# HelixDB/helix-db

Hardware: AMD Instinct MI355X
Metric: QPS @ recall@10>=0.95, 1Mx768 fp32; achieved HBM GB/s vs roofline (higher is better)
Workload: dtype f32; 1 GPU; configs[1]: 1000000x768 f32 per GPU, HNSW M=16/M0=32 ef_search=128 k=10, batch=1024 queries, squared-L2, strict-exhaustive beam (bit-exact vs reference CPU path), steps issued round-robin on 4 execution lanes; dataset=embedding, rows_per_gpu=1000000, rows_total=1000000, dim=768, batch=1024, k=10, ef_search=128, lanes=4, distinct_query_batches=25, exchange=single GPU, parallelism=1 GPU

## Files before the change

### helix-db_amd/csrc/hvx_api.hip

```cpp
#include <hip/hip_runtime.h>

#include <algorithm>
#include <atomic>
#include <cmath>
#include <cstdarg>
#include <cstdio>
#include <cstdlib>
#include <cstring>
#include <mutex>
#include <string>
#include <thread>
#include <vector>

#include "hvx_host.h"
#include "hvx_flat_mfma.h"
#include "hvx_hnsw_plan.h"

using namespace hvx;

namespace {
thread_local std::string g_err;
}

namespace hvx {
// ... 691 lines not shown
        return HVX_OK;
    }
    HIP_TRY(launch_validate_queries(ix->dev, d_queries, b, ix->limit, ix->d_qstatus, ix->d_qhdr, ix->stream));
    HnswArgs a;
    a.ix = ix->dev;
    a.queries = d_queries;
    a.qstatus = ix->d_qstatus;
    a.qhdr = ix->d_qhdr;
    a.bitmap = ix->d_bitmap;
    a.bitmap2 = (ad && ad->count_reads) ? ix->d_bitmap2 : nullptr;
    a.words_per_query = ix->words_per_query;
    a.k = k;
    a.ef = ef;
    a.out_ids = d_ids;
    a.out_scores = d_scores;
    a.out_counts = d_counts;
    a.out_status = d_status;
    a.qstats = d_qstats ? d_qstats : ix->d_qstats;
    a.tie_flags = ix->d_tie;
    a.rerun_list = ix->d_tie + ix->max_batch;
    a.rerun_ctl = ix->d_tie + 2 * (size_t)ix->max_batch;
    a.prof = nullptr;
    a.wave_clock = nullptr;
    a.adaptive = ad ? 1u : 0u;
    a.ad = ad ? *ad : AdaptArgs{};
    a.build_nodes = nullptr;
    a.build_ef_upper = 0;
    a.only_flagged = 0;
    a.occupancy = ix->occupancy;
    a.pair = ix->opt[HVX_OPT_HNSW_PAIR] >= 2u || (ix->opt[HVX_OPT_HNSW_PAIR] == 0u && ix->occupancy != 2u) ? 1u : 0u;
    a.pair_gatherers = ix->opt[HVX_OPT_HNSW_PAIR] == 3u ? 1u : 0u;
    a.log2cap = ix->opt[HVX_OPT_WAVE_LOG2CAP];
    a.shadow = nullptr;
    a.shadow_err = nullptr;
    if (ad) {
        if (!hnsw_wave_adaptive_supported(a))
            return fail(HVX_ERR_UNSUPPORTED, "the non-strict search arms serve f32 rows of any dimension / metric (bf16 rows: dim in "
                        "{128,256,384,512,768,1024,1536}, cosine / Euclidean), neighbour rows <= 64 ids, ef <= 800");
        if (ix->bitmap_dirty) {
            HIP_TRY(hipMemsetAsync(ix->d_bitmap, 0, (size_t)ix->max_batch * ix->words_per_query * 4, ix->stream));
            ix->bitmap_dirty = false;
        }
        const bool ad_prof = tuning_env("HVX_WAVE_PROF") != nullptr && hnsw_wave_supported(a) && ix->occupancy != 2u;
        if (ad_prof) {
            if (!ix->d_prof && ix->dalloc((void **)&ix->d_prof, (size_t)ix->max_batch * 80)) return HVX_ERR_DEVICE;
            a.prof = ix->d_prof;
        }
        hipEvent_t e0 = nullptr, e1 = nullptr;
        pick_events(ix, timed, &e0, &e1, &a.wave_clock);
        if (e0) HIP_TRY(hipEventRecord(e0, ix->stream));
        HIP_TRY(launch_hnsw_wave(a, b, ix->stream));
        if (e1) HIP_TRY(hipEventRecord(e1, ix->stream));
        if (ad_prof) {
            std::vector<unsigned long long> h((size_t)b * 10);
            HIP_TRY(hipMemcpyAsync(h.data(), ix->d_prof, h.size() * 8, hipMemcpyDeviceToHost, ix->stream));
            HIP_TRY(hipStreamSynchronize(ix->stream));
            double acc[10] = {0, 0, 0, 0, 0, 0, 0, 0, 0, 0};
            for (uint32_t i = 0; i < b; ++i)
                for (int j = 0; j < 10; ++j) acc[j] += (double)h[(size_t)i * 10 + j];
            fprintf(stderr, "[hvx prof, non-strict] per query: row-wait %.0f  visited-claim %.0f  decide+select %.0f  gather+fma %.0f  predict %.0f  admit %.0f  (layer-0 loop %.0f) cycles\n",
                    acc[0] / b, acc[1] / b, acc[6] / b, acc[2] / b, acc[3] / b, acc[4] / b, acc[7] / b);
        }
        return HVX_OK;
    }
    const bool prof = tuning_env("HVX_WAVE_PROF") != nullptr;
    if (prof) {
        if (!ix->d_prof && ix->dalloc((void **)&ix->d_prof, (size_t)ix->max_batch * 80)) return HVX_ERR_DEVICE;
        a.prof = ix->d_prof;
    }
    const bool force_general = ix->opt[HVX_OPT_HNSW_GENERAL_KERNEL] != 0;
    const bool wave = !(force_general && ix->dev.dtype == HVX_F32) && hnsw_wave_supported(a);
    if (!wave && ix->dev.dtype != HVX_F32)
        return fail(HVX_ERR_UNSUPPORTED, ix->dev.dtype == HVX_FP8_E4M3 ? "fp8 rows serve the exact scan only (HNSW over fp8 rows is not built)"
                    : "bf16 rows are served by the one-wavefront-per-query kernel only (dim in {128,256,384,512,768,1024,1536}, rows <= 64 ids, ef <= 800)");
    if (ix->bitmap_dirty) {
        HIP_TRY(hipMemsetAsync(ix->d_bitmap, 0, (size_t)ix->max_batch * ix->words_per_query * 4, ix->stream));
        ix->bitmap_dirty = false;
    }
    if (wave && (ix->occupancy == 2 || prof) && ix->dev.dtype == HVX_F32 && ix->dev.metric == kL2 && !ix->opt[HVX_OPT_HNSW_SHADOW_PRUNE]) {
        uint16_t *sh = nullptr;
        float *se = nullptr;
        int rc = shadow_catch_up(ix, &sh, &se);
        if (rc) return rc;
        a.shadow = sh;
        a.shadow_err = se;
    }
    hipEvent_t e0 = nullptr, e1 = nullptr;
    pick_events(ix, timed, &e0, &e1, &a.wave_clock);
    if (e0) HIP_TRY(hipEventRecord(e0, ix->stream));
    if (wave) {
        HIP_TRY(launch_hnsw_wave(a, b, ix->stream));
        if (prof) {
            std::vector<unsigned long long> h((size_t)b * 10);
            HIP_TRY(hipMemcpyAsync(h.data(), ix->d_prof, h.size() * 8, hipMemcpyDeviceToHost, ix->stream));
            HIP_TRY(hipStreamSynchronize(ix->stream));
            double acc[10] = {0, 0, 0, 0, 0, 0, 0, 0, 0, 0};
            for (uint32_t i = 0; i < b; ++i)
                for (int j = 0; j < 10; ++j) acc[j] += (double)h[(size_t)i * 10 + j];
            fprintf(stderr, "[hvx prof] per query: row-wait %.0f  visited+shadow %.0f  gather+fma %.0f  predict %.0f  admit %.0f  (layer-0 loop %.0f) cycles;"
                            " fresh-candidate predictions %.1f  row-prefetch hits %.1f;  full-beam rows: shadow-pruned %.1f  scored in f32 %.1f"
                            " (pruned share %.4f)\n",
                    acc[0] / b, acc[1] / b, acc[2] / b, acc[3] / b, acc[4] / b, acc[7] / b, acc[5] / b, acc[6] / b, acc[8] / b, acc[9] / b,
                    acc[8] + acc[9] > 0 ? acc[8] / (acc[8] + acc[9]) : 0.0);
        }
    } else {
        HIP_TRY(launch_hnsw_search(a, b, ix->stream));
        ix->bitmap_dirty = true;
    }
    if (e1) HIP_TRY(hipEventRecord(e1, ix->stream));
    return HVX_OK;
}

extern "C" int hvx_index_timing_begin(hvx_index *ix, uint32_t capacity) {
    if (!ix) return fail(HVX_ERR_INVARIANT, "null index");
    std::lock_guard<std::mutex> lock(ix->mu);
    HIP_TRY(hipSetDevice(ix->device));
    while (ix->ring.size() < (size_t)capacity * 2) {
        hipEvent_t e;
// ... 334 lines not shown
```

### helix-db_amd/csrc/hvx_flat_mfma.hip

```cpp
#include <hip/hip_runtime.h>

#include <algorithm>
#include <vector>

#include "hvx_hnsw_wave.h"
#include "hvx_host.h"
#include "hvx_flat_mfma.h"

using namespace hvx;

#define HIP_TRY(expr)                                                                              \
    do {                                                                                           \
        hipError_t _e = (expr);                                                                    \
        if (_e != hipSuccess) return fail(HVX_ERR_DEVICE, "%s: %s", #expr, hipGetErrorString(_e)); \
    } while (0)

namespace hvx {

constexpr int HVX_MFMA_FALLBACK = -1;

typedef __attribute__((ext_vector_type(8))) __bf16 bf16x8;
typedef __attribute__((ext_vector_type(16))) float f32x16;

__global__ __launch_bounds__(64) void bf16_row_norm2_kernel(const uint16_t *rows, uint32_t n, uint32_t dim, float *out) {
    const uint32_t r = blockIdx.x;
    if (r >= n) return;
    const uint16_t *p = rows + (size_t)r * dim;
    double acc = 0.0;
    for (uint32_t i = threadIdx.x; i < dim; i += 64) {
        const double v = (double)bf16_to_f32(p[i]);
        acc += v * v;
    }
    for (int s = 32; s > 0; s >>= 1) acc += __shfl_xor(acc, s, 64);
    if (threadIdx.x == 0) out[r] = (float)acc;
}

__global__ __launch_bounds__(64) void fp8_code_norm_kernel(const uint8_t *codes, uint32_t n, uint32_t dim, float *out) {
    const uint32_t r = blockIdx.x;
    if (r >= n) return;
    const uint8_t *p = codes + (size_t)r * dim;
    double acc = 0.0;
    for (uint32_t i = threadIdx.x; i < dim; i += 64) {
        const double v = (double)fp8_e4m3_decode(p[i]);
        acc += v * v;
    }
    for (int s = 32; s > 0; s >>= 1) acc += __shfl_xor(acc, s, 64);
    if (threadIdx.x == 0) out[r] = (float)sqrt(acc);
}

__global__ __launch_bounds__(256) void bf16_shadow_kernel(const float *rows, uint32_t ld, uint32_t dim, size_t cnt, uint16_t *out, float *err) {
    const uint32_t lane = threadIdx.x & 63u;
    for (size_t r = (size_t)blockIdx.x * 4 + (threadIdx.x >> 6); r < cnt; r += (size_t)gridDim.x * 4) {
        const float *x = rows + r * ld;
        uint16_t *o = out + r * dim;
        double acc = 0.0;
        if ((dim & 3u) == 0u) {
            for (uint32_t i = lane; i < dim / 4u; i += 64u) {
                const float4 v = reinterpret_cast<const float4 *>(x)[i];
                const uint32_t a = f32_to_bf16_rne(v.x), b = f32_to_bf16_rne(v.y), c = f32_to_bf16_rne(v.z), d = f32_to_bf16_rne(v.w);
                reinterpret_cast<uint2 *>(o)[i] = make_uint2(a | (b << 16), c | (d << 16));
                const double ea = (double)v.x - (double)bf16_to_f32((uint16_t)a), eb = (double)v.y - (double)bf16_to_f32((uint16_t)b);
                const double ec = (double)v.z - (double)bf16_to_f32((uint16_t)c), ed = (double)v.w - (double)bf16_to_f32((uint16_t)d);
                acc += ea * ea + eb * eb + ec * ec + ed * ed;
            }
        } else {
            for (uint32_t i = lane; i < dim; i += 64u) {
                const uint16_t h = f32_to_bf16_rne(x[i]);
                o[i] = h;
                const double ei = (double)x[i] - (double)bf16_to_f32(h);
                acc += ei * ei;
            }
        }
        for (int s = 32; s > 0; s >>= 1) acc += __shfl_xor(acc, s, 64);
        if (lane == 0u) {
            const double e = sqrt(acc) * (1.0 + 0x1p-30);
            float f = (float)e;
            if ((double)f < e) f = __uint_as_float(__float_as_uint(f) + 1u);
            err[r] = f;
        }
    }
}

__global__ __launch_bounds__(64) void split_queries_kernel(const float *q, uint32_t b, uint32_t bpad, uint32_t dim,
                                                           uint16_t *qhi, uint16_t *qlo, float *qn2, uint32_t fp8_layout,
                                                           uint16_t *qhi_tile8, uint32_t cosine) {
    const uint32_t r = blockIdx.x;
    if (r >= bpad) return;
    int qe = 0;
    if (cosine && r < b) {
        float mx = 0.f;
        for (uint32_t i = threadIdx.x; i < dim; i += 64) {
            const float v = q[(size_t)r * dim + i];
            if (f32_is_finite(v)) mx = fmaxf(mx, fabsf(v));
        }
        for (int s = 32; s > 0; s >>= 1) mx = fmaxf(mx, __shfl_xor(mx, s, 64));
        qe = cosine_query_exponent(mx);
    }
    double acc = 0.0;
    for (uint32_t i = threadIdx.x; i < dim; i += 64) {
        float v = r < b ? q[(size_t)r * dim + i] : 0.f;
        if (!f32_is_finite(v)) v = 0.f;
        if (qe) v = ldexpf(v, -qe);
        const uint16_t h = f32_to_bf16_rne(v);
        const float res = v - bf16_to_f32(h);
        const uint32_t s = fp8_layout == 2u ? i : (fp8_layout ? fp8_slot_of(i) : bf16_slot_of(i));
        qhi[(size_t)r * dim + s] = h;
        qlo[(size_t)r * dim + s] = f32_to_bf16_rne(res);
        if (qhi_tile8) qhi_tile8[(size_t)r * dim + tile_slot_fp8(s)] = h;
        acc += (double)v * (double)v;
    }
    for (int s = 32; s > 0; s >>= 1) acc += __shfl_xor(acc, s, 64);
    if (threadIdx.x == 0 && r < b) qn2[r] = (float)acc;
// ... 510 lines not shown
            const float t = t_thr;
            const float e = METRIC == kL2 ? a.erel * 0.5f * (a.qn2[q] + a.xmax2) : a.erel;
            const float kth = outn ? ss[outn - 1] : inf;
            ok = (outn == a.k && kth < t - e) ? 1u : 0u;
        }
        a.cert[q] = ok;
    }
}

template <uint32_t METRIC>
static hipError_t launch_rerank(const RerankArgs &a, uint32_t b, hipStream_t s) {
    const size_t lds = (size_t)a.ix.dim * 4 + 8192 + (a.sl_sc ? (size_t)a.sl_n * 4 : 0);
    switch (a.ix.dim >> 5) {
#define HVX_RR(N)                                                                                                   \
    case N:                                                                                                         \
        if (a.ix.dtype == HVX_FP8_E4M3) hipLaunchKernelGGL((rerank_bf16_kernel<METRIC, N, 1>), dim3(b), dim3(256), lds, s, a); \
        else if (a.ix.dtype == HVX_F32) hipLaunchKernelGGL((rerank_bf16_kernel<METRIC, N, 2>), dim3(b), dim3(256), lds, s, a);  \
        else hipLaunchKernelGGL((rerank_bf16_kernel<METRIC, N, 0>), dim3(b), dim3(256), lds, s, a);                  \
        break;
        HVX_RR(4) HVX_RR(8) HVX_RR(16) HVX_RR(24) HVX_RR(32) HVX_RR(48)
#undef HVX_RR
    default: return hipErrorInvalidValue;
    }
    return hipGetLastError();
}

}

extern "C" float hvxi_scan_error_bound(uint32_t kind, uint32_t l2, uint32_t dim) { return hvx::scan_error_bound(kind, l2 != 0u, dim); }
extern "C" int hvxi_cosine_query_exponent(float mx) { return hvx::cosine_query_exponent(mx); }
extern "C" uint32_t hvxi_cosine_term_trusted(float term) { return hvx::cosine_term_trusted(term) ? 1u : 0u; }

namespace hvx {

hipError_t launch_fp8_code_norm(const uint8_t *codes, uint32_t n, uint32_t dim, float *out, hipStream_t s) {
    if (n == 0) return hipSuccess;
    hipLaunchKernelGGL(fp8_code_norm_kernel, dim3(n), dim3(64), 0, s, codes, n, dim, out);
    return hipGetLastError();
}

hipError_t launch_bf16_row_norm2(const uint16_t *rows, uint32_t n, uint32_t dim, float *out, hipStream_t s) {
    if (n == 0) return hipSuccess;
    hipLaunchKernelGGL(bf16_row_norm2_kernel, dim3(n), dim3(64), 0, s, rows, n, dim, out);
    return hipGetLastError();
}

static int flat_mfma_impl(hvx_index *ix, const float *d_queries, uint32_t b, uint32_t k, const uint32_t *d_subset, uint32_t n_rows,
                          uint64_t *d_ids, float *d_scores, uint32_t *d_counts, uint32_t *d_status, bool timed, bool allow_filter,
                          bool force_tail = false);

int flat_mfma_device(hvx_index *ix, const float *d_queries, uint32_t b, uint32_t k, const uint32_t *d_subset, uint32_t n_rows,
                     uint64_t *d_ids, float *d_scores, uint32_t *d_counts, uint32_t *d_status, bool timed) {
    return flat_mfma_impl(ix, d_queries, b, k, d_subset, n_rows, d_ids, d_scores, d_counts, d_status, timed, true);
}

int shadow_catch_up(hvx_index *ix, uint16_t **shadow, float **err) {
    const DevIndex &d = ix->dev;
    hvx_image_shared &sh = *ix->shared;
    std::lock_guard<std::mutex> lock(sh.mu);
    *shadow = nullptr;
    *err = nullptr;
    if (sh.shadow_failed) return HVX_OK;
    if (!sh.shadow) {
        void *p = nullptr;
        const size_t rows_cap = std::max<uint64_t>(ix->cap_rows, d.n);
        const size_t sbytes = (rows_cap * d.dim * 2 + 15) / 16 * 16;
        if (hipMalloc(&p, std::max<size_t>(sbytes + rows_cap * 4, 16)) != hipSuccess) {
            (void)hipGetLastError();
            sh.shadow_failed = true;
            return HVX_OK;
        }
        sh.device = ix->device;
        sh.shadow = reinterpret_cast<uint16_t *>(p);
        sh.shadow_err = reinterpret_cast<float *>(reinterpret_cast<char *>(p) + sbytes);
        sh.shadow_rows = 0;
    }
    if (sh.shadow_rows < d.n) {
        const size_t r0 = sh.shadow_rows, cnt = d.n - r0;
        const uint32_t blocks = (uint32_t)std::min<size_t>((cnt + 3) / 4, 4096);
        hipLaunchKernelGGL(bf16_shadow_kernel, dim3(blocks), dim3(256), 0, ix->stream, d.vec + r0 * d.ld, d.ld, d.dim, cnt, sh.shadow + r0 * d.dim,
                           sh.shadow_err + r0);
        if (hipGetLastError() != hipSuccess || hipStreamSynchronize(ix->stream) != hipSuccess) return fail(HVX_ERR_DEVICE, "bf16 shadow conversion failed");
        sh.shadow_rows = d.n;
    }
    *shadow = sh.shadow;
    *err = sh.shadow_err;
    return HVX_OK;
}
static int ensure_shadow(hvx_index *ix) {
    uint16_t *s = nullptr;
    float *e = nullptr;
    const int rc = shadow_catch_up(ix, &s, &e);
    ix->m_shadow = s;
    return rc;
}

static int flat_mfma_impl(hvx_index *ix, const float *d_queries, uint32_t b, uint32_t k, const uint32_t *d_subset, uint32_t n_rows,
                          uint64_t *d_ids, float *d_scores, uint32_t *d_counts, uint32_t *d_status, bool timed, bool allow_filter,
                          bool force_tail) {
    const DevIndex &d = ix->dev;
    const uint32_t n = n_rows;
    if (k == 0) return fail(HVX_ERR_K_RANGE, "result count must be non-zero");
    if (k > 511) return fail(HVX_ERR_UNSUPPORTED, "bf16 exact scan supports k <= 511");
    const uint32_t nk = d.dim >> 5;
    if (nk != 4 && nk != 8 && nk != 16 && nk != 24 && nk != 32 && nk != 48)
        return fail(HVX_ERR_UNSUPPORTED, "bf16 / fp8 exact scan serves dim in {128,256,512,768,1024,1536}");
    HIP_TRY(launch_validate_queries(d, d_queries, b, ix->limit, ix->d_qstatus, ix->d_qhdr, ix->stream));
    if (n == 0) {
        if (timed) {
            HIP_TRY(hipEventRecord(ix->ev0, ix->stream));
            HIP_TRY(hipEventRecord(ix->ev1, ix->stream));
        }
        HIP_TRY(hipMemsetAsync(d_counts, 0, (size_t)b * 4, ix->stream));
        if (d_status) HIP_TRY(hipMemcpyAsync(d_status, ix->d_qstatus, (size_t)b * 4, hipMemcpyDeviceToDevice, ix->stream));
        return HVX_OK;
    }
    const uint32_t bpad = (b + 255u) / 256u * 256u;
    int rc;
    const bool fp8 = d.dtype == HVX_FP8_E4M3, f32 = d.dtype == HVX_F32;
    if ((size_t)bpad * d.dim > ix->cap_qsplit) {
        if ((rc = ix->regrow((void **)&ix->m_qhi, (size_t)bpad * d.dim * 2))) return rc;
        if ((rc = ix->regrow((void **)&ix->m_qlo, (size_t)bpad * d.dim * 2))) return rc;
        if (fp8 && (rc = ix->regrow((void **)&ix->m_qhi8, (size_t)bpad * d.dim * 2))) return rc;
        if ((rc = ix->regrow((void **)&ix->m_qn2, (size_t)bpad * 4))) return rc;
// ... 246 lines not shown
```

### helix-db_amd/csrc/hvx_hnsw_wave.h

```cpp
#pragma once
#include <type_traits>

#include "hvx_beam.h"
#include "hvx_device.h"
#include "hvx_hnsw_plan.h"
#include "hvx_kernels.h"
#include "hvx_shadow_bound.h"

namespace hvx {

constexpr uint32_t kTabEmpty = 0xFFFFFFFFu;
constexpr uint32_t kTentativeBit = 0x80000000u;
constexpr uint32_t kHashedBit = 0x40000000u;

__device__ __forceinline__ uint32_t umin_dpp_row(uint32_t v) {
    uint32_t t;
    t = (uint32_t)__builtin_amdgcn_mov_dpp((int)v, 0xB1, 0xF, 0xF, true); v = v < t ? v : t;
    t = (uint32_t)__builtin_amdgcn_mov_dpp((int)v, 0x4E, 0xF, 0xF, true); v = v < t ? v : t;
    t = (uint32_t)__builtin_amdgcn_mov_dpp((int)v, 0x141, 0xF, 0xF, true); v = v < t ? v : t;
    t = (uint32_t)__builtin_amdgcn_mov_dpp((int)v, 0x140, 0xF, 0xF, true); v = v < t ? v : t;
    return v;
}
__device__ __forceinline__ uint32_t wave_umin(uint32_t v) {
    v = umin_dpp_row(v);
// ... 183 lines not shown
                const uint32_t w0 = __float_as_uint(g.x[p][BF ? m : 0].x), w1 = __float_as_uint(g.x[p][BF ? m : 0].y);
                const float4 x0 = make_float4(__uint_as_float(w0 << 16), __uint_as_float(w0 & 0xFFFF0000u),
                                              __uint_as_float(w1 << 16), __uint_as_float(w1 & 0xFFFF0000u));
                fma_chunk<METRIC>(acc[p], q0, x0);
            }
#pragma unroll
            for (int p = 0; p < P; ++p) {
                const uint32_t w2 = __float_as_uint(g.x[p][BF ? m : 0].z), w3 = __float_as_uint(g.x[p][BF ? m : 0].w);
                const float4 x1 = make_float4(__uint_as_float(w2 << 16), __uint_as_float(w2 & 0xFFFF0000u),
                                              __uint_as_float(w3 << 16), __uint_as_float(w3 & 0xFFFF0000u));
                fma_chunk<METRIC>(acc[p], q1, x1);
            }
        }
    }
#pragma unroll
    for (int p = 0; p < P; ++p) {
        float r = avx_tree_reduce(acc[p]);
        if (METRIC == kCosine) {
            const uint32_t nd = node[p];
            r = cosine_finish_fn(r, qhdr, g.h[p], [&]() {
                if (BF) {
                    const uint16_t *rb = ix.vecb + (size_t)nd * ix.dim;
                    return stable_half_cosine_fn(ix.dim, [&](uint32_t i) { return qglobal[i]; },
                                                 [&](uint32_t i) { return bf16_to_f32(rb[bf16_slot_of(i)]); });
                }
                const float *rf = ix.vec + (size_t)nd * ix.ld;
                return stable_half_cosine_fn(ix.dim, [&](uint32_t i) { return qglobal[i]; }, [&](uint32_t i) { return rf[i]; });
            });
        }
        out[p] = r;
    }
}



template <uint32_t RW> struct QueryRngT {
    static constexpr uint32_t kBlocks = RW / 16u;
    uint32_t *buf;
    uint32_t key[8];
    uint32_t base;
    uint32_t pos;
    bool ready;

    __device__ __forceinline__ void seed(uint64_t state) {
        const uint64_t MUL = 6364136223846793005ULL, INC = 11634580027462260723ULL;
#pragma unroll
        for (int i = 0; i < 8; ++i) {
            state = state * MUL + INC;
            const uint32_t xs = (uint32_t)(((state >> 18) ^ state) >> 27), rot = (uint32_t)(state >> 59);
            key[i] = (xs >> rot) | (xs << ((32u - rot) & 31u));
        }
        base = 0;
        pos = 0;
        ready = false;
    }
    __device__ __forceinline__ void ensure(int lane) {
        if (ready && pos + 66u <= base + RW) return;
        base = pos & ~15u;
        const uint32_t ctr = (base >> 4) + (uint32_t)lane;
        uint32_t st[16] = {0x61707865u, 0x3320646eu, 0x79622d32u, 0x6b206574u, key[0], key[1], key[2], key[3],
                           key[4], key[5], key[6], key[7], ctr, 0u, 0u, 0u};
        uint32_t x[16];
#pragma unroll
        for (int i = 0; i < 16; ++i) x[i] = st[i];
#define HVX_QR(a, b, c, d)                                                                                   \
    x[a] += x[b]; x[d] = __builtin_rotateleft32(x[d] ^ x[a], 16); x[c] += x[d]; x[b] = __builtin_rotateleft32(x[b] ^ x[c], 12); \
// ... 221 lines not shown
                const uint32_t f = f0 + (uint32_t)grp;
                const float d = generic_distance(fr_id[f < nf ? f : f0]);
                if (f < nf && j == 0) fr_d[f] = d;
            }
            __syncthreads();
            return;
        }
        while (f0 < nf) {
            const uint32_t rem = nf - f0;
            if (kWide4 && rem > 24u * P) { pass(std::integral_constant<int, kWide4 ? 4 * P : P>{}, f0, nf); f0 += 32u * P; }
            else if (kWide4 && rem > 16u * P) { pass(std::integral_constant<int, kWide4 ? 3 * P : P>{}, f0, nf); f0 += 24u * P; }
            else if (kWide2 && rem > 8u * P) { pass(std::integral_constant<int, kWide2 ? 2 * P : P>{}, f0, nf); f0 += 16u * P; }
            else { pass(std::integral_constant<int, P>{}, f0, nf); f0 += 8u * P; }
        }
        __syncthreads();
    };
    auto score_one = [&](uint32_t node) __attribute__((always_inline)) -> float {
        if constexpr (GEN) {
            return __uint_as_float(__builtin_amdgcn_readlane(__float_as_uint(generic_distance(node)), 0));
        } else {
            uint32_t nd[1] = {node};
            float o[1];
            Gather<NK, 1, BF> g;
            gather_issue<NK, 1, BF, 1, METRIC == kCosine>(ix, nd, slot, g);
            gather_consume<METRIC, NK, 1, BF>(ix, qs, g, nd, slot, qhdr, qglobal, o);
            return __uint_as_float(__builtin_amdgcn_readlane(__float_as_uint(o[0]), 0));
        }
    };
    constexpr bool SP = !AD && !BUILD && !BF && !GEN && METRIC == kL2 && R <= 6 && (OCC == 2 || PROF);
    constexpr int SL = SP ? NK / 2 : 1;
    constexpr int kFL = (kWide4 ? 4 * P : (kWide2 ? 2 * P : P)) * NL;
    constexpr int kSWmax = !SP ? 1 : 8 * SL * 4 <= kFL * 3 ? 8 : 4 * SL * 4 <= kFL * 3 ? 4 : 3 * SL * 4 <= kFL * 3 ? 3 : 2 * SL * 4 <= kFL * 3 ? 2 : 1;
    const bool shadow_on = SP && a.shadow != nullptr;
    auto shadow_pass = [&](auto width, uint32_t f0, uint32_t nf) __attribute__((always_inline)) {
        constexpr int W = decltype(width)::value;
        uint32_t nd[W];
        uint4 x[W][SL];
        float e[W];
#pragma unroll
        for (int p = 0; p < W; ++p) {
            const uint32_t f = f0 + (uint32_t)(p * 8 + grp);
            nd[p] = fr_id[f < nf ? f : f0];
        }
#pragma unroll
        for (int p = 0; p < W; ++p) e[p] = a.shadow_err[nd[p]];
#pragma unroll
        for (int p = 0; p < W; ++p) {
            const uint4 *rp = reinterpret_cast<const uint4 *>(a.shadow + (size_t)nd[p] * ix.dim) + j;
#pragma unroll
            for (int k = 0; k < SL; ++k) x[p][k] = rp[k * 8];
        }
        __builtin_amdgcn_sched_barrier(0);
        float4 acc[W];
#pragma unroll
        for (int p = 0; p < W; ++p) acc[p] = make_float4(0.f, 0.f, 0.f, 0.f);
        const float4 *qp = reinterpret_cast<const float4 *>(qs) + 2 * j;
#pragma unroll
        for (int k = 0; k < SL; ++k) {
            const float4 q0 = qp[16 * k], q1 = qp[16 * k + 1];
#pragma unroll
            for (int p = 0; p < W; ++p) {
                const uint4 w = x[p][k];
                fma_chunk<kL2>(acc[p], q0, make_float4(__uint_as_float(w.x << 16), __uint_as_float(w.x & 0xFFFF0000u),
                                                       __uint_as_float(w.y << 16), __uint_as_float(w.y & 0xFFFF0000u)));
                fma_chunk<kL2>(acc[p], q1, make_float4(__uint_as_float(w.z << 16), __uint_as_float(w.z & 0xFFFF0000u),
                                                       __uint_as_float(w.w << 16), __uint_as_float(w.w & 0xFFFF0000u)));
            }
        }
#pragma unroll
        for (int p = 0; p < W; ++p) {
            float r = (acc[p].x + acc[p].y) + (acc[p].z + acc[p].w);
            r += __shfl_xor(r, 1, 8);
            r += __shfl_xor(r, 2, 8);
            r += __shfl_xor(r, 4, 8);
            const uint32_t f = f0 + (uint32_t)(p * 8 + grp);
            if (f < nf && j == 0) fr_d[f] = shadow_l2_lower_bound(r, e[p], ix.dim);
        }
    };
    auto shadow_prune = [&](uint32_t nf, float thr) __attribute__((always_inline)) -> uint32_t {
        if constexpr (SP) {
            uint32_t f0 = 0;
            while (f0 < nf) {
                const uint32_t rem = nf - f0;
                if (kSWmax >= 8 && rem > 32u) { shadow_pass(std::integral_constant<int, kSWmax >= 8 ? 8 : 1>{}, f0, nf); f0 += 64u; }
                else if (kSWmax >= 4 && rem > 24u) { shadow_pass(std::integral_constant<int, kSWmax >= 4 ? 4 : 1>{}, f0, nf); f0 += 32u; }
                else if (kSWmax >= 3 && rem > 16u) { shadow_pass(std::integral_constant<int, kSWmax >= 3 ? 3 : 1>{}, f0, nf); f0 += 24u; }
                else if (kSWmax >= 2 && rem > 8u) { shadow_pass(std::integral_constant<int, kSWmax >= 2 ? 2 : 1>{}, f0, nf); f0 += 16u; }
                else { shadow_pass(std::integral_constant<int, 1>{}, f0, nf); f0 += 8u; }
            }
            __syncthreads();
            const bool in = (uint32_t)lane < nf;
            const uint32_t id = in ? fr_id[lane] : kSentinel;
            const bool keep = in && !(fr_d[in ? lane : 0] > thr);
            const unsigned long long km = __ballot(keep);
            __syncthreads();
            if (keep) fr_id[__builtin_popcountll(km & ((1ull << lane) - 1ull))] = id;
            __syncthreads();
            return (uint32_t)__builtin_popcountll(km);
        } else {
            return nf;
        }
    };
    auto frontier_from = [&](uint32_t nid, uint32_t &deg) __attribute__((always_inline)) -> uint32_t {
        const bool valid = nid != kSentinel;
        const bool isnew = V.insert(nid, valid, lane);
        const unsigned long long um = __ballot(isnew);
        deg = (uint32_t)__builtin_popcountll(__ballot(valid));
        if (isnew) fr_id[__builtin_popcountll(um & ((1ull << lane) - 1ull))] = nid;
        __syncthreads();
// ... 429 lines not shown
```

### helix-db_amd/csrc/hvx_host.h

```cpp
#pragma once
#include <hip/hip_runtime.h>

#include <algorithm>
#include <atomic>
#include <cstdlib>
#include <memory>
#include <mutex>
#include <vector>

#include "hvx_csr_view.h"
#include "hvx_kernels.h"
#include "hvx_walk_core.h"

struct hvx_allocs {
    int device = 0;
    std::vector<void *> v;
    ~hvx_allocs() {
        if (v.empty()) return;
        (void)hipSetDevice(device);
        for (void *p : v) (void)hipFree(p);
    }
};

struct hvx_image_shared {
    std::mutex mu;
    int device = 0;
    uint16_t *shadow = nullptr;
    uint32_t shadow_rows = 0;
    float *shadow_err = nullptr;
    bool shadow_failed = false;
    uint64_t *dir_code = nullptr;
    uint32_t *dir_row = nullptr;
    uint32_t *dir_prefix = nullptr;
    const uint64_t *dir_for = nullptr;
    uint32_t dir_rows = 0;
    uint64_t visible_seq = 0;
    uint32_t v_n = 0, v_entry = 0, v_max_layer = 0, v_has_entry = 0;
    std::shared_ptr<const std::vector<uint8_t>> v_dead;
    uint32_t v_n_dead = 0;
    const uint32_t *v_dead_dev = nullptr;
    std::shared_ptr<const std::vector<uint8_t>> dir_dead;
    uint64_t vec_epoch = 0;
    std::atomic<uint64_t> rewrite_epoch{0};
    uint64_t v_entry_point = 0;
    bool v_contiguous = true;
    std::shared_ptr<const std::vector<uint64_t>> v_ids;
    ~hvx_image_shared() {
        if (shadow || dir_code || dir_row) (void)hipSetDevice(device);
        if (shadow) (void)hipFree(shadow);
        if (dir_code) (void)hipFree(dir_code);
        if (dir_row) (void)hipFree(dir_row);
        if (dir_prefix) (void)hipFree(dir_prefix);
    }
};

struct hvx_index {
    int device = 0;
    hvx_index_desc desc{};
    hvx::DevIndex dev{};
    float limit = 0.f;
    uint32_t max_batch = 1024;
    uint32_t words_per_query = 0;
// ... 131 lines not shown
        }
        auto it = std::lower_bound(ids.begin(), ids.end(), id);
        if (it == ids.end() || *it != id) return hvx::kSentinel;
        return (uint32_t)(it - ids.begin());
    }
};

namespace hvx {
#ifdef HVX_TUNING
inline const char *tuning_env(const char *name) { return getenv(name); }
#else
inline const char *tuning_env(const char *) { return nullptr; }
#endif
int fail(int code, const char *fmt, ...);
int import_index(const hvx_index_desc *desc, const uint64_t *node_ids, const float *vectors, const uint64_t *l0_offsets,
                 const uint64_t *l0_neighbors, const uint16_t *level, const uint64_t *up_offsets, const uint64_t *up_neighbors,
                 uint32_t min_s0, uint32_t min_su, hvx_index **out, uint64_t reserve_rows = 0, uint64_t reserve_up_rows = 0);
int check_k_ef(uint32_t k, uint32_t ef);
int enqueue_search(const hvx_index *ix, const float *d_queries, uint32_t b, uint32_t k, uint32_t ef, uint64_t *d_ids,
                   float *d_scores, uint32_t *d_counts, uint32_t *d_status, hvx_query_stats *d_qstats, bool timed,
                   const AdaptArgs *ad = nullptr);
int enqueue_search_params(hvx_index *ix, const float *d_queries, uint32_t b, const hvx_search_params *params, uint64_t *d_ids, float *d_scores,
                          uint32_t *d_counts, uint32_t *d_status);
int collect_stats(hvx_index *ix, uint32_t b, const hvx_query_stats *d_qstats, hvx_stats *stats);
float component_limit(uint32_t metric, uint32_t dim);
int flat_scan_device(hvx_index *ix, const float *d_queries, uint32_t b, uint32_t k, const uint32_t *d_subset,
                     uint32_t n_rows, uint64_t *d_ids, float *d_scores, uint32_t *d_counts, uint32_t *d_status,
                     bool timed);
bool flat_scan_on_matrix_cores(const hvx_index *ix, uint32_t b, uint32_t k, uint32_t n_rows);
int flat_scan_valu(hvx_index *ix, const float *d_queries, uint32_t b, uint32_t k, const uint32_t *d_subset, uint32_t n_rows,
                   uint64_t *d_ids, float *d_scores, uint32_t *d_counts, uint32_t *d_status, bool timed, bool record_begin);
int flat_mfma_device(hvx_index *ix, const float *d_queries, uint32_t b, uint32_t k, const uint32_t *d_subset, uint32_t n_rows,
                     uint64_t *d_ids, float *d_scores, uint32_t *d_counts, uint32_t *d_status, bool timed);
int shadow_catch_up(hvx_index *ix, uint16_t **shadow, float **err);
struct RestrictedPlan {
    uint32_t strategy;
    walk::Plan p;
};
int restricted_make_plan(const hvx_restricted_params &rp, uint64_t candidates, uint32_t dim, RestrictedPlan *out, const hvx_index *ix = nullptr);
void restricted_sample_ranks(uint64_t candidates, uint32_t count, std::vector<uint64_t> &out);
int restricted_run_plan(hvx_index *ix, const float *queries, uint32_t b, uint32_t k_stride, const RestrictedPlan &plan, const uint32_t *d_rows,
                        uint32_t n_rows, const uint32_t *d_samples, uint64_t *out_ids, float *out_scores, uint32_t *out_counts,
                        uint32_t *out_status, hvx_restricted_stats *rstats, hvx_stats *stats);
hipError_t launch_bf16_row_norm2(const uint16_t *rows, uint32_t n, uint32_t dim, float *out, hipStream_t s);
hipError_t launch_fp8_code_norm(const uint8_t *codes, uint32_t n, uint32_t dim, float *out, hipStream_t s);
int flat_scan_host(hvx_index *ix, const float *queries, uint32_t b, uint32_t k, const uint32_t *d_subset,
                   uint32_t n_rows, uint64_t *out_ids, float *out_scores, uint32_t *out_counts,
                   uint32_t *out_status, hvx_stats *stats);
bool restricted_direct_supported(const hvx_index *ix, uint32_t k);
bool restricted_direct_pays(const hvx_index *ix, uint32_t k, uint32_t lists, uint64_t longest);
bool restricted_older_serves(const hvx_index *ix, uint32_t k);
hipError_t restricted_direct_launch_wide4(const void *args, bool ext, bool unrolled, hipStream_t s);
hipError_t restricted_direct_launch_wide13(const void *args, bool ext, bool unrolled, hipStream_t s);
int restricted_direct_enqueue(hvx_index *ix, const float *d_queries, uint32_t b, uint32_t k, uint32_t k_stride, const uint32_t *d_rows,
                              uint32_t n_rows, const uint64_t *d_ext_ids, const uint64_t *d_offsets, uint32_t max_set, uint64_t *d_ids,
                              float *d_scores, uint32_t *d_counts, uint32_t *d_status, const uint32_t *d_lens = nullptr, uint32_t ext_stride = 0,
                              const uint32_t *d_n_rows = nullptr);
int restricted_direct_shared_devcount(hvx_index *ix, const float *queries, uint32_t b, uint32_t k, const uint32_t *d_rows, uint32_t rows_cap,
                                      const uint32_t *d_counters, uint64_t *out_ids, float *out_scores, uint32_t *out_counts, uint32_t *out_status,
                                      uint64_t *out_candidates, hvx_restricted_stats *rstats, hvx_stats *stats);
int restricted_direct_lists_devlens(hvx_index *ix, const float *queries, uint32_t b, uint32_t k, const uint64_t *d_ids, uint32_t stride,
                                    const uint32_t *d_ctl, size_t ctl_words, uint64_t *out_ids, float *out_scores, uint32_t *out_counts,
                                    uint32_t *out_status, hvx_stats *stats);
struct PathListsArgs {
    CsrView g;
    const uint32_t *seeds, *seed_off;
    uint32_t n_hops, direction[16], label_off[17];
// ... 47 lines not shown
```

### helix-db_amd/csrc/hvx_kernels.h

```cpp
#pragma once
#include <hip/hip_runtime.h>
#include <stdint.h>

#include "../../include/helix_vec.h"
#include "hvx_device.h"

namespace hvx {

struct AdaptArgs {
    const uint64_t *node_hash;
    const uint64_t *qhash;
    const float *thr_break;
    hvx_adaptive_stats *stats;
    uint32_t filtering;
    uint32_t configured;
    uint32_t sampling;
    float ratio;
    float pre_override;
    uint32_t count_reads;
    uint32_t read_budget;
    uint32_t bypass_windowed;
    uint32_t min_frontier, window_expansions;
    float min_filter_rate;
};

struct HnswArgs {
    DevIndex ix;
    const float *queries;
    const uint32_t *qstatus;
    const float *qhdr;
    uint32_t *bitmap;
    uint32_t *bitmap2;
    uint32_t words_per_query;
    uint32_t k, ef;
    uint64_t *out_ids;
    float *out_scores;
    uint32_t *out_counts;
    uint32_t *out_status;
    hvx_query_stats *qstats;
    uint32_t *tie_flags;
    uint32_t *rerun_list;
    uint32_t *rerun_ctl;
    unsigned long long *prof;
    unsigned long long *wave_clock;
    uint32_t adaptive;
    const uint32_t *build_nodes;
    uint32_t build_ef_upper;
    uint32_t *tie_count;
    uint32_t only_flagged;
    uint32_t occupancy;
    uint32_t pair;
    uint32_t pair_gatherers;
    uint32_t log2cap;
    const uint16_t *shadow;
    const float *shadow_err;
    AdaptArgs ad;
};

size_t hnsw_lds_bytes(uint32_t ld);
hipError_t launch_hnsw_search(const HnswArgs &a, uint32_t b, hipStream_t s);
hipError_t launch_simhash_rows(const float *planes_t, const float *rows, uint32_t dim, uint32_t ld, uint64_t n, uint64_t *out,
                               hipStream_t s);
hipError_t launch_simhash_rows_bf16(const float *planes_t, const uint16_t *rows, uint32_t dim, uint64_t n, uint64_t *out,
                                    hipStream_t s);
void simhash_planes_transposed(uint32_t dim, uint64_t seed, float *planes_t);
hipError_t launch_hnsw_wave(const HnswArgs &a, uint32_t b, hipStream_t s);

hipError_t launch_validate_queries(const DevIndex &ix, const float *d_queries, uint32_t b, float limit,
                                   uint32_t *d_status, float *d_qhdr, hipStream_t s);

hipError_t launch_validate_rows(const DevIndex &ix, uint32_t n, float limit, uint32_t *d_status, float *d_hdr,
                                hipStream_t s);

hipError_t launch_round_bf16_inplace(float *v, size_t count, hipStream_t s);
hipError_t launch_pack_bf16(const float *staging, uint16_t *dst, uint32_t n, uint32_t dim, hipStream_t s);
hipError_t launch_quantize_fp8(float *staging, uint8_t *dst, float *rowscale, uint32_t n, uint32_t dim, hipStream_t s);
hipError_t launch_read_rows(const DevIndex &ix, uint64_t row0, uint64_t n, float *out, hipStream_t s);
hipError_t launch_f32_row_norm2(const float *rows, uint32_t n, uint32_t ld, uint32_t dim, float *out, hipStream_t s);

struct FlatArgs {
    DevIndex ix;
    const float *queries;
    const uint32_t *qstatus;
    const float *qhdr;
    const uint32_t *subset;
    uint32_t n_rows;
    uint32_t row0, rows;
    float *dist;
// ... 23 lines not shown
```

### helix-db_amd/csrc/hvx_shadow_bound.h

```cpp
#pragma once
#include <stdint.h>

#if defined(__HIPCC__)
#define HVX_SB_HD __host__ __device__ __forceinline__
#else
#include <math.h>
#define HVX_SB_HD inline
#endif

namespace hvx {

constexpr float kNoBound = -1.0f;

HVX_SB_HD float shadow_l2_lower_bound(float st, float e, uint32_t n) {
    if (!(st >= 0.0f) || !(e >= 0.0f)) return kNoBound;
    const float ub = sqrtf(st) * (1.0f + 0x1p-10f) + e + 1.0f;
    const float U = ub * ub * (1.0f + 0x1p-10f);
    if (!(U <= 0x1p126f)) return kNoBound;
    if (st < 0x1p-40f) return 0.0f;
    const float c = 1.0f - (float)(n + 3u) * 0x1p-23f;
    const float r3 = sqrtf(st * c) * (1.0f - 0x1p-19f);
    if (!(r3 > e)) return 0.0f;
    const float r4 = r3 - e;
    const float r7 = (r4 * r4 * c) * (1.0f - 0x1p-20f);
    return r7 >= 0x1p-60f ? r7 : 0.0f;
}

}
```

Before: 1.408 million queries/s.

## Score bf16 shadow rows with packed dot2 and a dot-product lower bound

```diff
diff --git a/helix-db_amd/csrc/hvx_api.hip b/helix-db_amd/csrc/hvx_api.hip
--- a/helix-db_amd/csrc/hvx_api.hip
+++ b/helix-db_amd/csrc/hvx_api.hip
@@ -747,7 +747,7 @@
     a.pair_gatherers = ix->opt[HVX_OPT_HNSW_PAIR] == 3u ? 1u : 0u;
     a.log2cap = ix->opt[HVX_OPT_WAVE_LOG2CAP];
     a.shadow = nullptr;
-    a.shadow_err = nullptr;
+    a.shadow_rec = nullptr;
     if (ad) {
         if (!hnsw_wave_adaptive_supported(a))
             return fail(HVX_ERR_UNSUPPORTED, "the non-strict search arms serve f32 rows of any dimension / metric (bf16 rows: dim in "
@@ -794,11 +794,11 @@
     }
     if (wave && (ix->occupancy == 2 || prof) && ix->dev.dtype == HVX_F32 && ix->dev.metric == kL2 && !ix->opt[HVX_OPT_HNSW_SHADOW_PRUNE]) {
         uint16_t *sh = nullptr;
-        float *se = nullptr;
+        float2 *se = nullptr;
         int rc = shadow_catch_up(ix, &sh, &se);
         if (rc) return rc;
         a.shadow = sh;
-        a.shadow_err = se;
+        a.shadow_rec = se;
     }
     hipEvent_t e0 = nullptr, e1 = nullptr;
     pick_events(ix, timed, &e0, &e1, &a.wave_clock);
diff --git a/helix-db_amd/csrc/hvx_flat_mfma.hip b/helix-db_amd/csrc/hvx_flat_mfma.hip
--- a/helix-db_amd/csrc/hvx_flat_mfma.hip
+++ b/helix-db_amd/csrc/hvx_flat_mfma.hip
@@ -48,36 +48,38 @@
     if (threadIdx.x == 0) out[r] = (float)sqrt(acc);
 }
 
-__global__ __launch_bounds__(256) void bf16_shadow_kernel(const float *rows, uint32_t ld, uint32_t dim, size_t cnt, uint16_t *out, float *err) {
+__global__ __launch_bounds__(256) void bf16_shadow_kernel(const float *rows, uint32_t ld, uint32_t dim, size_t cnt, uint16_t *out, float2 *rec) {
     const uint32_t lane = threadIdx.x & 63u;
     for (size_t r = (size_t)blockIdx.x * 4 + (threadIdx.x >> 6); r < cnt; r += (size_t)gridDim.x * 4) {
         const float *x = rows + r * ld;
         uint16_t *o = out + r * dim;
-        double acc = 0.0;
+        double acc = 0.0, nx = 0.0;
         if ((dim & 3u) == 0u) {
             for (uint32_t i = lane; i < dim / 4u; i += 64u) {
                 const float4 v = reinterpret_cast<const float4 *>(x)[i];
                 const uint32_t a = f32_to_bf16_rne(v.x), b = f32_to_bf16_rne(v.y), c = f32_to_bf16_rne(v.z), d = f32_to_bf16_rne(v.w);
                 reinterpret_cast<uint2 *>(o)[i] = make_uint2(a | (b << 16), c | (d << 16));
-                const double ea = (double)v.x - (double)bf16_to_f32((uint16_t)a), eb = (double)v.y - (double)bf16_to_f32((uint16_t)b);
-                const double ec = (double)v.z - (double)bf16_to_f32((uint16_t)c), ed = (double)v.w - (double)bf16_to_f32((uint16_t)d);
+                const double ya = (double)bf16_to_f32((uint16_t)a), yb = (double)bf16_to_f32((uint16_t)b);
+                const double yc = (double)bf16_to_f32((uint16_t)c), yd = (double)bf16_to_f32((uint16_t)d);
+                const double ea = (double)v.x - ya, eb = (double)v.y - yb, ec = (double)v.z - yc, ed = (double)v.w - yd;
                 acc += ea * ea + eb * eb + ec * ec + ed * ed;
+                nx += ya * ya + yb * yb + yc * yc + yd * yd;
             }
         } else {
             for (uint32_t i = lane; i < dim; i += 64u) {
                 const uint16_t h = f32_to_bf16_rne(x[i]);
                 o[i] = h;
-                const double ei = (double)x[i] - (double)bf16_to_f32(h);
+                const double yi = (double)bf16_to_f32(h), ei = (double)x[i] - yi;
                 acc += ei * ei;
-            }
-        }
-        for (int s = 32; s > 0; s >>= 1) acc += __shfl_xor(acc, s, 64);
-        if (lane == 0u) {
-            const double e = sqrt(acc) * (1.0 + 0x1p-30);
-            float f = (float)e;
-            if ((double)f < e) f = __uint_as_float(__float_as_uint(f) + 1u);
-            err[r] = f;
-        }
+                nx += yi * yi;
+            }
+        }
+        for (int s = 32; s > 0; s >>= 1) {
+            acc += __shfl_xor(acc, s, 64);
+            nx += __shfl_xor(nx, s, 64);
+        }
+        if (lane == 0u)
+            rec[r] = make_float2(shadow_dot_round(sqrt(acc) * (1.0 + 0x1p-30), true), shadow_dot_round(nx * (1.0 - 0x1p-30), false));
     }
 }
 
@@ -654,6 +656,75 @@
 extern "C" uint32_t hvxi_cosine_term_trusted(float term) { return hvx::cosine_term_trusted(term) ? 1u : 0u; }
 
 namespace hvx {
+template <int W, int SL>
+__global__ __launch_bounds__(64) void shadow_dot_probe_kernel(const float *queries, const uint16_t *shadow, uint32_t rpq, float *out_d, float *out_c) {
+    constexpr uint32_t dim = (uint32_t)SL * 64u;
+    __shared__ __attribute__((aligned(16))) float qs[dim];
+    const int lane = (int)threadIdx.x, grp = lane >> 3, j = lane & 7;
+    const float *qg = queries + (size_t)blockIdx.x * dim;
+    for (uint32_t i = (uint32_t)lane; i < dim / 4u; i += 64) reinterpret_cast<float4 *>(qs)[i] = reinterpret_cast<const float4 *>(qg)[i];
+    const ShadowDotQuery c = shadow_dot_const(shadow_dot_query_stage(qg, dim, lane));
+    if (lane == 0) reinterpret_cast<float4 *>(out_c)[blockIdx.x] = make_float4(c.nq, c.qn, c.rho, c.p);
+    __syncthreads();
+    const uint16_t *rows = shadow + (size_t)blockIdx.x * rpq * dim;
+    for (uint32_t f0 = 0; f0 < rpq; f0 += 8u * W) {
+        uint4 x[W][SL];
+        float d[W];
+#pragma unroll
+        for (int p = 0; p < W; ++p) {
+            const uint32_t f = f0 + (uint32_t)(p * 8 + grp);
+            const uint4 *rp = reinterpret_cast<const uint4 *>(rows + (size_t)(f < rpq ? f : f0) * dim) + j;
+#pragma unroll
+            for (int k = 0; k < SL; ++k) x[p][k] = rp[k * 8];
+        }
+        shadow_dot_rows<W, SL>(x, qs, j, d);
+#pragma unroll
+        for (int p = 0; p < W; ++p) {
+            const uint32_t f = f0 + (uint32_t)(p * 8 + grp);
+            if (f < rpq && j == 0) out_d[(size_t)blockIdx.x * rpq + f] = d[p];
+        }
+    }
+}
+template <int W> static hipError_t launch_shadow_dot_probe(uint32_t dim, uint32_t nq, uint32_t rpq, const float *q, const uint16_t *sh, float *d, float *c) {
+    if (dim == 128u) hipLaunchKernelGGL((shadow_dot_probe_kernel<W, 2>), dim3(nq), dim3(64), 0, nullptr, q, sh, rpq, d, c);
+    else if (dim == 768u) hipLaunchKernelGGL((shadow_dot_probe_kernel<W, 12>), dim3(nq), dim3(64), 0, nullptr, q, sh, rpq, d, c);
+    else hipLaunchKernelGGL((shadow_dot_probe_kernel<W, 24>), dim3(nq), dim3(64), 0, nullptr, q, sh, rpq, d, c);
+    return hipGetLastError();
+}
+}
+extern "C" int hvxi_shadow_dot_probe(const float *queries, const float *rows, uint32_t nq, uint32_t rpq, uint32_t dim, uint32_t width, float *d, float *rec,
+                                     float *consts) {
+    if (!queries || !rows || !d || !rec || !consts || nq == 0u || rpq == 0u || nq > 4096u || rpq > 4096u) return fail(HVX_ERR_INVARIANT, "shadow dot probe: bad arguments");
+    if ((dim != 128u && dim != 768u && dim != 1536u) || width < 1u || width > 3u) return fail(HVX_ERR_UNSUPPORTED, "shadow dot probe: dim in {128, 768, 1536}, width 1..3");
+    const size_t n = (size_t)nq * rpq, qb = (size_t)nq * dim * 4, xb = n * dim * 4, sb = n * dim * 2;
+    char *buf = nullptr;
+    const size_t o_x = (qb + 255) / 256 * 256, o_s = o_x + (xb + 255) / 256 * 256, o_r = o_s + (sb + 255) / 256 * 256, o_d = o_r + (n * 8 + 255) / 256 * 256,
+                 o_c = o_d + (n * 4 + 255) / 256 * 256, total = o_c + (size_t)nq * 16;
+    HIP_TRY(hipMalloc((void **)&buf, total));
+    hipError_t e = hipMemcpy(buf, queries, qb, hipMemcpyHostToDevice);
+    if (e == hipSuccess) e = hipMemcpy(buf + o_x, rows, xb, hipMemcpyHostToDevice);
+    if (e == hipSuccess) {
+        hipLaunchKernelGGL(bf16_shadow_kernel, dim3((uint32_t)std::min<size_t>((n + 3) / 4, 4096)), dim3(256), 0, nullptr, reinterpret_cast<const float *>(buf + o_x), dim,
+                           dim, n, reinterpret_cast<uint16_t *>(buf + o_s), reinterpret_cast<float2 *>(buf + o_r));
+        e = hipGetLastError();
+    }
+    if (e == hipSuccess) {
+        const float *q = reinterpret_cast<const float *>(buf);
+        const uint16_t *sh = reinterpret_cast<const uint16_t *>(buf + o_s);
+        float *dd = reinterpret_cast<float *>(buf + o_d), *dc = reinterpret_cast<float *>(buf + o_c);
+        e = width == 1u ? launch_shadow_dot_probe<1>(dim, nq, rpq, q, sh, dd, dc)
+          : width == 2u ? launch_shadow_dot_probe<2>(dim, nq, rpq, q, sh, dd, dc) : launch_shadow_dot_probe<3>(dim, nq, rpq, q, sh, dd, dc);
+    }
+    if (e == hipSuccess) e = hipDeviceSynchronize();
+    if (e == hipSuccess) e = hipMemcpy(d, buf + o_d, n * 4, hipMemcpyDeviceToHost);
+    if (e == hipSuccess) e = hipMemcpy(rec, buf + o_r, n * 8, hipMemcpyDeviceToHost);
+    if (e == hipSuccess) e = hipMemcpy(consts, buf + o_c, (size_t)nq * 16, hipMemcpyDeviceToHost);
+    (void)hipFree(buf);
+    if (e != hipSuccess) return fail(HVX_ERR_DEVICE, "shadow dot probe: %s", hipGetErrorString(e));
+    return HVX_OK;
+}
+
+namespace hvx {
 
 hipError_t launch_fp8_code_norm(const uint8_t *codes, uint32_t n, uint32_t dim, float *out, hipStream_t s) {
     if (n == 0) return hipSuccess;
@@ -676,42 +747,42 @@
     return flat_mfma_impl(ix, d_queries, b, k, d_subset, n_rows, d_ids, d_scores, d_counts, d_status, timed, true);
 }
 
-int shadow_catch_up(hvx_index *ix, uint16_t **shadow, float **err) {
+int shadow_catch_up(hvx_index *ix, uint16_t **shadow, float2 **rec) {
     const DevIndex &d = ix->dev;
     hvx_image_shared &sh = *ix->shared;
     std::lock_guard<std::mutex> lock(sh.mu);
     *shadow = nullptr;
-    *err = nullptr;
+    *rec = nullptr;
     if (sh.shadow_failed) return HVX_OK;
     if (!sh.shadow) {
         void *p = nullptr;
         const size_t rows_cap = std::max<uint64_t>(ix->cap_rows, d.n);
         const size_t sbytes = (rows_cap * d.dim * 2 + 15) / 16 * 16;
-        if (hipMalloc(&p, std::max<size_t>(sbytes + rows_cap * 4, 16)) != hipSuccess) {
+        if (hipMalloc(&p, std::max<size_t>(sbytes + rows_cap * 8, 16)) != hipSuccess) {
             (void)hipGetLastError();
             sh.shadow_failed = true;
             return HVX_OK;
         }
         sh.device = ix->device;
         sh.shadow = reinterpret_cast<uint16_t *>(p);
-        sh.shadow_err = reinterpret_cast<float *>(reinterpret_cast<char *>(p) + sbytes);
+        sh.shadow_rec = reinterpret_cast<float2 *>(reinterpret_cast<char *>(p) + sbytes);
         sh.shadow_rows = 0;
     }
     if (sh.shadow_rows < d.n) {
         const size_t r0 = sh.shadow_rows, cnt = d.n - r0;
         const uint32_t blocks = (uint32_t)std::min<size_t>((cnt + 3) / 4, 4096);
         hipLaunchKernelGGL(bf16_shadow_kernel, dim3(blocks), dim3(256), 0, ix->stream, d.vec + r0 * d.ld, d.ld, d.dim, cnt, sh.shadow + r0 * d.dim,
-                           sh.shadow_err + r0);
+                           sh.shadow_rec + r0);
         if (hipGetLastError() != hipSuccess || hipStreamSynchronize(ix->stream) != hipSuccess) return fail(HVX_ERR_DEVICE, "bf16 shadow conversion failed");
         sh.shadow_rows = d.n;
     }
     *shadow = sh.shadow;
-    *err = sh.shadow_err;
+    *rec = sh.shadow_rec;
     return HVX_OK;
 }
 static int ensure_shadow(hvx_index *ix) {
     uint16_t *s = nullptr;
-    float *e = nullptr;
+    float2 *e = nullptr;
     const int rc = shadow_catch_up(ix, &s, &e);
     ix->m_shadow = s;
     return rc;
diff --git a/helix-db_amd/csrc/hvx_hnsw_wave.h b/helix-db_amd/csrc/hvx_hnsw_wave.h
--- a/helix-db_amd/csrc/hvx_hnsw_wave.h
+++ b/helix-db_amd/csrc/hvx_hnsw_wave.h
@@ -239,6 +239,73 @@
     }
 }
 
+
+typedef __bf16 hvx_bf16x2 __attribute__((ext_vector_type(2)));
+typedef float hvx_f32x2 __attribute__((ext_vector_type(2)));
+__device__ __forceinline__ float dot2_bf16(uint32_t a, uint32_t b, float c) {
+    return __builtin_amdgcn_fdot2_f32_bf16(__builtin_bit_cast(hvx_bf16x2, a), __builtin_bit_cast(hvx_bf16x2, b), c, false);
+}
+__device__ __forceinline__ uint32_t shadow_dot_pack(float a, float b) {
+    const hvx_f32x2 v = {a, b};
+    return __builtin_bit_cast(uint32_t, __builtin_convertvector(v, hvx_bf16x2));
+}
+__device__ __forceinline__ float shadow_dot_query_stage(const float *qglobal, uint32_t dim, int lane) {
+    double q2 = 0.0, r2 = 0.0;
+    for (uint32_t i = (uint32_t)lane; i < dim / 4u; i += 64) {
+        const float4 v = reinterpret_cast<const float4 *>(qglobal)[i];
+        const float in[4] = {v.x, v.y, v.z, v.w};
+        const uint32_t h[2] = {shadow_dot_pack(v.x, v.y), shadow_dot_pack(v.z, v.w)};
+#pragma unroll
+        for (int c = 0; c < 4; ++c) {
+            const double y = (double)bf16_to_f32((uint16_t)(h[c >> 1] >> (16 * (c & 1)))), r = (double)in[c] - y;
+            q2 += y * y;
+            r2 += r * r;
+        }
+    }
+    for (int s = 32; s > 0; s >>= 1) {
+        q2 += __shfl_xor(q2, s, 64);
+        r2 += __shfl_xor(r2, s, 64);
+    }
+    const ShadowDotQuery c = shadow_dot_query(q2, r2, dim);
+    return lane == 0 ? c.nq : lane == 1 ? c.qn : lane == 2 ? c.rho : c.p;
+}
+__device__ __forceinline__ ShadowDotQuery shadow_dot_const(float packed) {
+    const uint32_t u = __float_as_uint(packed);
+    return ShadowDotQuery{__uint_as_float(__builtin_amdgcn_readlane(u, 0)), __uint_as_float(__builtin_amdgcn_readlane(u, 1)),
+                          __uint_as_float(__builtin_amdgcn_readlane(u, 2)), __uint_as_float(__builtin_amdgcn_readlane(u, 3))};
+}
+template <int W, int SL>
+__device__ __forceinline__ void shadow_dot_rows(const uint4 (&x)[W][SL], const float *qs, int j, float (&out)[W]) {
+    constexpr int C = W >= 2 ? 2 : 4;
+    float acc[W][C];
+#pragma unroll
+    for (int p = 0; p < W; ++p)
+#pragma unroll
+        for (int c = 0; c < C; ++c) acc[p][c] = 0.f;
+    const float4 *qp = reinterpret_cast<const float4 *>(qs) + 2 * j;
+#pragma unroll
+    for (int k = 0; k < SL; ++k) {
+        const float4 q0 = qp[16 * k], q1 = qp[16 * k + 1];
+        const uint32_t l0 = shadow_dot_pack(q0.x, q0.y), l1 = shadow_dot_pack(q0.z, q0.w);
+        const uint32_t l2 = shadow_dot_pack(q1.x, q1.y), l3 = shadow_dot_pack(q1.z, q1.w);
+#pragma unroll
+        for (int p = 0; p < W; ++p) {
+            const uint4 w = x[p][k];
+            acc[p][0] = dot2_bf16(w.x, l0, acc[p][0]);
+            acc[p][1] = dot2_bf16(w.y, l1, acc[p][1]);
+            acc[p][C - 2] = dot2_bf16(w.z, l2, acc[p][C - 2]);
+            acc[p][C - 1] = dot2_bf16(w.w, l3, acc[p][C - 1]);
+        }
+    }
+#pragma unroll
+    for (int p = 0; p < W; ++p) {
+        float r = C == 4 ? (acc[p][0] + acc[p][1]) + (acc[p][C - 2] + acc[p][C - 1]) : acc[p][0] + acc[p][1];
+        r += __shfl_xor(r, 1, 8);
+        r += __shfl_xor(r, 2, 8);
+        r += __shfl_xor(r, 4, 8);
+        out[p] = r;
+    }
+}
 
 
 template <uint32_t RW> struct QueryRngT {
@@ -526,18 +593,23 @@
     constexpr int kFL = (kWide4 ? 4 * P : (kWide2 ? 2 * P : P)) * NL;
     constexpr int kSWmax = !SP ? 1 : 8 * SL * 4 <= kFL * 3 ? 8 : 4 * SL * 4 <= kFL * 3 ? 4 : 3 * SL * 4 <= kFL * 3 ? 3 : 2 * SL * 4 <= kFL * 3 ? 2 : 1;
     const bool shadow_on = SP && a.shadow != nullptr;
+    float sqv = 0.f;
+    if constexpr (SP) {
+        if (shadow_on) sqv = shadow_dot_query_stage(qglobal, (uint32_t)NK * 32u, lane);
+    }
     auto shadow_pass = [&](auto width, uint32_t f0, uint32_t nf) __attribute__((always_inline)) {
         constexpr int W = decltype(width)::value;
         uint32_t nd[W];
         uint4 x[W][SL];
-        float e[W];
+        float2 rec[W];
+        float d[W];
 #pragma unroll
         for (int p = 0; p < W; ++p) {
             const uint32_t f = f0 + (uint32_t)(p * 8 + grp);
             nd[p] = fr_id[f < nf ? f : f0];
         }
 #pragma unroll
-        for (int p = 0; p < W; ++p) e[p] = a.shadow_err[nd[p]];
+        for (int p = 0; p < W; ++p) rec[p] = a.shadow_rec[nd[p]];
 #pragma unroll
         for (int p = 0; p < W; ++p) {
             const uint4 *rp = reinterpret_cast<const uint4 *>(a.shadow + (size_t)nd[p] * ix.dim) + j;
@@ -545,30 +617,12 @@
             for (int k = 0; k < SL; ++k) x[p][k] = rp[k * 8];
         }
         __builtin_amdgcn_sched_barrier(0);
-        float4 acc[W];
-#pragma unroll
-        for (int p = 0; p < W; ++p) acc[p] = make_float4(0.f, 0.f, 0.f, 0.f);
-        const float4 *qp = reinterpret_cast<const float4 *>(qs) + 2 * j;
-#pragma unroll
-        for (int k = 0; k < SL; ++k) {
-            const float4 q0 = qp[16 * k], q1 = qp[16 * k + 1];
-#pragma unroll
-            for (int p = 0; p < W; ++p) {
-                const uint4 w = x[p][k];
-                fma_chunk<kL2>(acc[p], q0, make_float4(__uint_as_float(w.x << 16), __uint_as_float(w.x & 0xFFFF0000u),
-                                                       __uint_as_float(w.y << 16), __uint_as_float(w.y & 0xFFFF0000u)));
-                fma_chunk<kL2>(acc[p], q1, make_float4(__uint_as_float(w.z << 16), __uint_as_float(w.z & 0xFFFF0000u),
-                                                       __uint_as_float(w.w << 16), __uint_as_float(w.w & 0xFFFF0000u)));
-            }
-        }
+        shadow_dot_rows<W, SL>(x, qs, j, d);
+        const ShadowDotQuery sq = shadow_dot_const(sqv);
 #pragma unroll
         for (int p = 0; p < W; ++p) {
-            float r = (acc[p].x + acc[p].y) + (acc[p].z + acc[p].w);
-            r += __shfl_xor(r, 1, 8);
-            r += __shfl_xor(r, 2, 8);
-            r += __shfl_xor(r, 4, 8);
             const uint32_t f = f0 + (uint32_t)(p * 8 + grp);
-            if (f < nf && j == 0) fr_d[f] = shadow_l2_lower_bound(r, e[p], ix.dim);
+            if (f < nf && j == 0) fr_d[f] = shadow_dot_lower_bound(d[p], sq, rec[p].x, rec[p].y, ix.dim);
         }
     };
     auto shadow_prune = [&](uint32_t nf, float thr) __attribute__((always_inline)) -> uint32_t {
diff --git a/helix-db_amd/csrc/hvx_host.h b/helix-db_amd/csrc/hvx_host.h
--- a/helix-db_amd/csrc/hvx_host.h
+++ b/helix-db_amd/csrc/hvx_host.h
@@ -27,7 +27,7 @@
     int device = 0;
     uint16_t *shadow = nullptr;
     uint32_t shadow_rows = 0;
-    float *shadow_err = nullptr;
+    float2 *shadow_rec = nullptr;
     bool shadow_failed = false;
     uint64_t *dir_code = nullptr;
     uint32_t *dir_row = nullptr;
@@ -225,7 +225,7 @@
                    uint64_t *d_ids, float *d_scores, uint32_t *d_counts, uint32_t *d_status, bool timed, bool record_begin);
 int flat_mfma_device(hvx_index *ix, const float *d_queries, uint32_t b, uint32_t k, const uint32_t *d_subset, uint32_t n_rows,
                      uint64_t *d_ids, float *d_scores, uint32_t *d_counts, uint32_t *d_status, bool timed);
-int shadow_catch_up(hvx_index *ix, uint16_t **shadow, float **err);
+int shadow_catch_up(hvx_index *ix, uint16_t **shadow, float2 **rec);
 struct RestrictedPlan {
     uint32_t strategy;
     walk::Plan p;
diff --git a/helix-db_amd/csrc/hvx_kernels.h b/helix-db_amd/csrc/hvx_kernels.h
--- a/helix-db_amd/csrc/hvx_kernels.h
+++ b/helix-db_amd/csrc/hvx_kernels.h
@@ -53,7 +53,7 @@
     uint32_t pair_gatherers;
     uint32_t log2cap;
     const uint16_t *shadow;
-    const float *shadow_err;
+    const float2 *shadow_rec;
     AdaptArgs ad;
 };
 
diff --git a/helix-db_amd/csrc/hvx_shadow_bound.h b/helix-db_amd/csrc/hvx_shadow_bound.h
--- a/helix-db_amd/csrc/hvx_shadow_bound.h
+++ b/helix-db_amd/csrc/hvx_shadow_bound.h
@@ -26,4 +26,64 @@
     return r7 >= 0x1p-60f ? r7 : 0.0f;
 }
 
+struct ShadowDotQuery {
+    float nq;
+    float qn;
+    float rho;
+    float p;
+};
+
+HVX_SB_HD uint16_t shadow_dot_piece(float q) {
+    union { float f; uint32_t u; } a;
+    a.f = q;
+    return (uint16_t)((a.u + 0x7FFFu + ((a.u >> 16) & 1u)) >> 16);
 }
+
+HVX_SB_HD float shadow_dot_round(double v, bool up) {
+    float f = (float)v;
+    union { float f; uint32_t u; } w;
+    w.f = f;
+    if (up && (double)f < v) w.u += 1u;
+    if (!up && (double)f > v && w.u != 0u) w.u = (w.u == 0x7F800000u) ? 0x7F7FFFFFu : w.u - 1u;
+    return w.f;
+}
+
+HVX_SB_HD ShadowDotQuery shadow_dot_query(double q2, double r2, uint32_t n) {
+    ShadowDotQuery c;
+    c.nq = shadow_dot_round(q2 * (1.0 - 0x1p-30), false);
+    c.qn = shadow_dot_round(sqrt(q2) * (1.0 + 0x1p-30), true);
+    c.rho = shadow_dot_round(sqrt(r2) * (1.0 + 0x1p-30), true);
+    c.p = shadow_dot_round(0x1p-125 * ((double)(3u * n + 128u) + 2.0 * (double)n * (double)c.qn) * (1.0 + 0x1p-40), true);
+    return c;
+}
+
+HVX_SB_HD float shadow_dot_sx(float nx) { return sqrtf(nx) * (1.0f + 0x1p-19f) + 0x1p-73f; }
+
+HVX_SB_HD float shadow_dot_error(const ShadowDotQuery &c, float sx, uint32_t n) {
+    const float g = (float)((3u * n + 7u) / 8u + 16u) * 0x1p-23f * (1.0f + 0x1p-7f);
+    return ((g * c.qn) * sx + (c.p + ((float)n * 0x1p-124f) * sx)) * (1.0f + 0x1p-19f);
+}
+
+HVX_SB_HD float shadow_dot_lower_bound(float D, const ShadowDotQuery &c, float rec_e, float rec_nx, uint32_t n) {
+    if (n > 4096u || !(rec_e >= 0.0f) || !(rec_nx >= 0.0f) || !(c.nq >= 0.0f) || !(c.qn >= 0.0f) || !(c.rho >= 0.0f) || !(c.p >= 0x1p-118f)) return kNoBound;
+    if (!(D >= -0x1.fffffep127f && D <= 0x1.fffffep127f)) return kNoBound;
+    const float sx = shadow_dot_sx(rec_nx);
+    const float ee = (rec_e + c.rho) * (1.0f + 0x1p-23f);
+    const float ub = c.qn + sx + ee + 1.0f;
+    const float U = ub * ub * (1.0f + 0x1p-10f);
+    if (!(U <= 0x1p126f)) return kNoBound;
+    const float t1 = (c.nq + rec_nx) * (1.0f - 0x1p-23f);
+    const float u = D + shadow_dot_error(c, sx, n);
+    const float u1 = u + 0x1p-22f * (u < 0.0f ? -u : u);
+    const float st = (t1 - 2.0f * u1) * (1.0f - 0x1p-23f);
+    if (!(st <= 0x1p126f)) return kNoBound;
+    if (!(st >= 0x1p-40f)) return 0.0f;
+    const float c1 = 1.0f - (float)(n + 3u) * 0x1p-23f;
+    const float r3 = sqrtf(st) * (1.0f - 0x1p-19f);
+    if (!(r3 > ee)) return 0.0f;
+    const float r4 = r3 - ee;
+    const float r7 = (r4 * r4 * c1) * (1.0f - 0x1p-20f);
+    return r7 >= 0x1p-60f ? r7 : 0.0f;
+}
+
+}
```

After: 1.475 million queries/s, median of 6. 1.05x the previous value.
